# miroslavradojevic/pnr

Hardware: AMD Instinct MI355X
Metric: Mvox/s traced (Frangi+SMC step) on 1024^3 synthetic stack; % HBM roofline (higher is better)
Workload: dtype f32 (+f64 3x3 eigen-solver)

## Files before the change

### pnr_amd/csrc/api.cpp

```cpp
#include "ctx.h"
#include "replay.h"
#include "stream_sched.h"
#include "../host/reconstruct.h"
#include "recon.h"
#include "volume.h"
#include "radius.h"
#include "filter.h"
#include "distance.h"
#include <algorithm>
#include <cfloat>
#include <cmath>
#include <cstdlib>
#include <cstring>
#include <numeric>
#include <unordered_map>
#include <fstream>
#include <thread>
#include <sched.h>

namespace pnr {
static thread_local char g_err[512] = "";
void set_error(const char *fmt, ...)
{
    va_list ap;
// ... 964 lines not shown
    o.lag = std::max(-1, lag);
    pnr::SchedStats st;
    std::string err;
    const int rc = pnr::run_stream(eng, seeds, n, p->ni, o, sh, r, &st, err);
    if (rc) { set_error("%s", err.c_str()); return rc; }
    *n_nodes = (int64_t)r.nodes.size();
    *n_links = (int64_t)r.links.size() / 2;
    if (nodes) std::memcpy(nodes, r.nodes.data(), sizeof(pnr_node) * (size_t)std::min<int64_t>(cap_nodes, *n_nodes));
    if (links) std::memcpy(links, r.links.data(), 8 * (size_t)std::min<int64_t>(cap_links, *n_links));
    if (n_traces_used) *n_traces_used = r.trace_count;
    if (n_iterations) *n_iterations = st.iters;
    return PNR_OK;
}

namespace {
struct OptEntry { const char *key; int pnr::Options::*i32; int64_t pnr::Options::*i64; int64_t lo, hi; };
const OptEntry OPTS[] = {
    {"window", &pnr::Options::window, nullptr, 0, 1 << 20},      {"look0", &pnr::Options::look0, nullptr, 0, 1 << 24},
    {"look_pct", &pnr::Options::look_pct, nullptr, -1, 100000},   {"poll", &pnr::Options::poll, nullptr, 0, 1024},
    {"groups", &pnr::Options::groups, nullptr, 0, 4},            {"split_x10", &pnr::Options::split_x10, nullptr, 0, 10000},
    {"max_split", &pnr::Options::max_split, nullptr, 1, 4096},   {"stash_mb", nullptr, &pnr::Options::stash_mb, 1, 1 << 20},
    {"host_threads", &pnr::Options::host_threads, nullptr, 0, 1024}, {"local_ranks", &pnr::Options::local_ranks, nullptr, 1, 1024},
    {"trace_timing", &pnr::Options::trace_timing, nullptr, 0, 1}, {"seed_timing", &pnr::Options::seed_timing, nullptr, 0, 1},
    {"trace_log", &pnr::Options::trace_log, nullptr, 0, 1},
    {"replay_batches", &pnr::Options::replay_batches, nullptr, 0, 1}, {"batch_growth", &pnr::Options::batch_growth, nullptr, 100, 100000},
    {"batch_max", &pnr::Options::batch_max, nullptr, 1, 1 << 24}, {"no_stash", &pnr::Options::no_stash, nullptr, 0, 1},
    {"exchange_block", nullptr, &pnr::Options::exchange_block, 0, 1 << 28}, {"frangi_prune", &pnr::Options::frangi_prune, nullptr, 0, 1},
    {"cube_copy", &pnr::Options::cube_copy, nullptr, 0, 1},      {"gauss_march", &pnr::Options::gauss_march, nullptr, 0, 1},
    {"tentative", &pnr::Options::tentative, nullptr, 0, 1},      {"target", &pnr::Options::target, nullptr, -1, 1 << 20},
    {"sums_deep", &pnr::Options::sums_deep, nullptr, -1, 1},      {"sums_deep_max", &pnr::Options::sums_deep_max, nullptr, 0, 1 << 20},
    {"lag", &pnr::Options::lag, nullptr, -1, 1023},               {"profile_every", &pnr::Options::profile_every, nullptr, 1, 1024},
    {"overfill", &pnr::Options::overfill, nullptr, 0, 1},        {"concentrate", &pnr::Options::concentrate, nullptr, 0, 100},
    {"share_scales", &pnr::Options::share_scales, nullptr, 0, 1}, {"share_min", &pnr::Options::share_min, nullptr, 0, 1 << 20},
    {"hess_chunk", &pnr::Options::hess_chunk, nullptr, 0, 1 << 20},
    {"dist_split", &pnr::Options::dist_split, nullptr, 0, 1 << 22}, {"dist_pairs_per_launch", nullptr, &pnr::Options::dist_pairs_per_launch, 0, 1ll << 44},
};
}

int pnr_set_option(pnr_ctx *c, const char *key, int64_t value)
{
    PNR_REQUIRE(c && key, PNR_E_ARG, "null argument");
    if (std::strcmp(key, "recon_timing") == 0) {
        PNR_REQUIRE(value == 0 || value == 1, PNR_E_ARG, "option recon_timing = %lld outside [0, 1]", (long long)value);
        advantra::set_recon_timing(value != 0);
        return PNR_OK;
    }
    for (const OptEntry &e : OPTS)
        if (std::strcmp(e.key, key) == 0) {
            PNR_REQUIRE(value >= e.lo && value <= e.hi, PNR_E_ARG, "option %s = %lld outside [%lld, %lld]", key, (long long)value, (long long)e.lo, (long long)e.hi);
            if (e.i32) c->opt.*(e.i32) = (int)value; else c->opt.*(e.i64) = value;
            return PNR_OK;
        }
    set_error("unknown option '%s'", key);
    return PNR_E_ARG;
}

int pnr_get_option(pnr_ctx *c, const char *key, int64_t *value)
{
    PNR_REQUIRE(c && key && value, PNR_E_ARG, "null argument");
    if (std::strcmp(key, "recon_timing") == 0) { *value = advantra::recon_timing() ? 1 : 0; return PNR_OK; }
    if (std::strcmp(key, "host_threads_effective") == 0) { *value = pnr::host_threads(c->opt); return PNR_OK; }
    if (std::strcmp(key, "frangi_recomputes") == 0) { *value = c->frangi_recomputes; return PNR_OK; }
    for (const OptEntry &e : OPTS)
        if (std::strcmp(e.key, key) == 0) {
            *value = e.i32 ? (int64_t)(c->opt.*(e.i32)) : c->opt.*(e.i64);
            return PNR_OK;
        }
// ... 195 lines not shown
```

### pnr_amd/csrc/ctx.h

```cpp
#pragma once
#include "../../include/pnr_hip.h"
#include "../../include/pnr_hip_test.h"
#include "devbuf.h"
#include <hip/hip_runtime.h>
#include <algorithm>
#include <cstdarg>
#include <cstdio>
#include <map>
#include <string>
#include <unordered_map>
#include <vector>

namespace pnr {

void set_error(const char *fmt, ...);

#define PNR_HIP(call)                                                                        \
    do {                                                                                     \
        hipError_t e_ = (call);                                                              \
        if (e_ != hipSuccess) {                                                              \
            pnr::set_error("%s failed: %s (%s:%d)", #call, hipGetErrorString(e_), __FILE__, __LINE__); \
            return PNR_E_HIP;                                                                \
        }                                                                                    \
    } while (0)
// ... 33 lines not shown
void find_scale_pairs(Tables &t);
void glibc_rand_stream(uint32_t seed, int n, uint32_t *out);
int gaussian_taps(float sig, std::vector<float> &g);

struct Options {
    int window = 0;
    int look0 = 0, look_pct = -1;
    int target = -1;
    int sums_deep = -1;
    int sums_deep_max = 96;
    int lag = -1;
    int concentrate = 1;
    int overfill = 1;
    int poll = 0;
    int groups = 0;
    int split_x10 = 0;
    int max_split = 96;
    int64_t stash_mb = 65536;
    int host_threads = 0;
    int local_ranks = 1;
    int trace_timing = 0, seed_timing = 0;
    int profile_every = 1;
    int trace_log = 0;
    int replay_batches = 0;
    int batch_growth = 200, batch_max = 1024;
    int no_stash = 0;
    int frangi_prune = 1;
    int hess_chunk = 0;
    int tentative = 1;
    int gauss_march = 1;
    int cube_copy = 1;
    int share_scales = 1;
    int share_min = 0;
    int dist_split = 0;
    int64_t dist_pairs_per_launch = 0;
    int64_t exchange_block = 0;
};
int host_threads(const Options &o);

struct KernelTimer {
    double ms = 0;
    int64_t launches = 0;
};

}

struct pnr_ctx {
    pnr_params prm;
    pnr::Options opt;
    int device = 0;
    hipStream_t own_stream = nullptr, stream = nullptr;
    pnr::Tables tab;

    int64_t w = 0, h = 0, l = 0, N = 0;
    const uint8_t *d_img = nullptr;
    pnr::DevBuf<uint8_t> d_img_owned;

    pnr::DevBuf<float> d_tmpA, d_tmpB, d_J;
    pnr::DevBuf<uint8_t> d_Vx, d_Vy, d_Vz, d_J8;
    pnr::DevBuf<unsigned int> d_minmax;
    pnr::DevBuf<float> d_F[PNR_MAX_SIGMAS];
    pnr::DevBuf<uint8_t> d_scale;
    bool frangi_pruned = false, frangi_exact_once = false;
    float Jmax_run = 0.f;
    int64_t frangi_recomputes = 0;
    int64_t fr_zs0 = 0, fr_zs1 = 0;
// ... 160 lines not shown
```

### pnr_amd/csrc/smc_device.h

```cpp
#pragma once
#include "ctx.h"
#include <cfloat>
#include <cmath>

namespace {
typedef long long i64;
typedef float f32x2 __attribute__((ext_vector_type(2)));

struct Vol {
    const unsigned char *img;
    int w, h, l;
    i64 wh;
    float xmax, ymax, zmax;
};

struct Tab {
    const float *p, *u, *w0, *w0cws, *v, *w, *wcws;
    const float4 *tmpl;
    const int *M, *moff;
    const float *corrc, *sig;
    const unsigned int *rng;
    int sz, ndir, nsig, Mtot;
};

// ... 408 lines not shown
            const bool more = (iv * nu + iu + 1) < nv * nu;
            const float *nxt = more ? wk : wk - nw;
            r_wd = nxt[lane < nw ? lane : 0];
            for (int iw0 = 0; iw0 < nw; iw0 += G) {
                float xs[G], ys[G], zs[G];
#pragma unroll
                for (int j = 0; j < G; j++) {
                    const int iw = (iw0 + j < nw) ? iw0 + j : nw - 1;
                    const float ww = bcast(r_aw, iw);
                    const f32x2 xy = (f32x2){x1, y1} + (f32x2){ww, ww} * (f32x2){f.wx, f.wy};
                    xs[j] = xy.x;
                    ys[j] = xy.y;
                    zs[j] = z1 + ww * f.wz;
                }
                const Samples<G> sm = interp_group<G, CS>(V, B, xs, ys, zs);
#pragma unroll
                for (int j = 0; j < G; j++)
                    if (iw0 + j < nw) {
                        const float di = sm.v[j] - ag;
                        corra += di * bcast(r_cur, iw0 + j);
                        corrb = (float)((double)corrb + (double)di * (double)di);
                    }
            }
        }
    }
    }
    const float prod = corrb * corrc;
    return (prod > FLT_MIN) ? corra / sqrtf(prod) : 0.f;
}

template <int CS, bool IS2D = false, bool FAST = false, int PITCH = CS, bool INVOL = false>
__device__ __forceinline__ void sample_slice(const Vol &V, const Box &B, const Frame &f, int nv, int nu, int nw,
                                             const float *__restrict__ ax, int iv, float *__restrict__ stash_wave, int iu0 = 0,
                                             int iu1 = 1 << 30)
{
    constexpr int G = CHAIN_G;
    const int lane = threadIdx.x & 63;
    const float r_au = ax[nv + (lane < nu ? lane : 0)];
    const float r_aw = ax[nv + nu + (lane < nw ? lane : 0)];
    const float vv = ax[iv];
    const float x0 = f.px + vv * f.nvx, y0 = f.py + vv * f.nvy, z0 = f.pz + vv * f.nvz;
    if (iu1 > nu) iu1 = nu;
    typedef __attribute__((address_space(1))) float gfloat;
    gfloat *sp;
    {
        const unsigned long long a = (unsigned long long)(stash_wave + ((i64)iv * nu + iu0) * nw * 64);
        sp = (gfloat *)(((unsigned long long)(unsigned)__builtin_amdgcn_readfirstlane((int)(a >> 32)) << 32) | (unsigned)__builtin_amdgcn_readfirstlane((int)a));
    }
    const unsigned ulane = (unsigned)lane;
    for (int iu = iu0; iu < iu1; ++iu) {
        const float uu = bcast(r_au, iu);
        const float x1 = x0 + uu * f.ux, y1 = y0 + uu * f.uy, z1 = z0 + uu * f.uz;
        int iw0 = 0;
        for (; iw0 + G <= nw; iw0 += G) {
            float xs[G], ys[G], zs[G];
#pragma unroll
            for (int j = 0; j < G; j++) {
                const float ww = bcast(r_aw, iw0 + j);
                const f32x2 xy = (f32x2){x1, y1} + (f32x2){ww, ww} * (f32x2){f.wx, f.wy};
                xs[j] = xy.x;
                ys[j] = xy.y;
                zs[j] = z1 + ww * f.wz;
            }
            const Samples<G> sm = interp_group<G, CS, IS2D, FAST, PITCH, INVOL>(V, B, xs, ys, zs);
            gfloat *const pl = (sp + iw0 * 64) + ulane;
#pragma unroll
            for (int j = 0; j < G; j++) STASH_ST(&pl[j * 64], sm.v[j]);
        }
        if (iw0 < nw) {
            float xs[G], ys[G], zs[G];
#pragma unroll
            for (int j = 0; j < G; j++) {
                const int iw = (iw0 + j < nw) ? iw0 + j : nw - 1;
                const float ww = bcast(r_aw, iw);
                const f32x2 xy = (f32x2){x1, y1} + (f32x2){ww, ww} * (f32x2){f.wx, f.wy};
                xs[j] = xy.x;
                ys[j] = xy.y;
                zs[j] = z1 + ww * f.wz;
            }
            const Samples<G> sm = interp_group<G, CS, IS2D, FAST, PITCH, INVOL>(V, B, xs, ys, zs);
#pragma unroll
            for (int j = 0; j < G; j++)
                if (iw0 + j < nw) STASH_ST(&((sp + iw0 * 64) + ulane)[j * 64], sm.v[j]);
        }
        sp += nw * 64;
    }
}

template <int CS, bool IS2D = false, bool FAST = false, int PITCH = CS, bool INVOL = false>
__device__ __forceinline__ void sample_slice_packed(const Vol &V, const Box &B, const Frame &f, int nv, int nu, int nw,
                                                    const float *__restrict__ ax, int iv, int parts, int p, bool active,
                                                    float *__restrict__ stash_col, int stride, int r0 = 0, int r1 = 1 << 30)
{
    constexpr int G = CHAIN_G;
    const int lane = threadIdx.x & 63;
    const float r_au = ax[nv + (lane < nu ? lane : 0)];
    const float r_aw = ax[nv + nu + (lane < nw ? lane : 0)];
    const float vv = ax[iv];
    const float x0 = f.px + vv * f.nvx, y0 = f.py + vv * f.nvy, z0 = f.pz + vv * f.nvz;
    int rows = (nu + parts - 1) / parts;
    if (r1 < rows) rows = r1;
    for (int r = r0; r < rows; ++r) {
        const int iu = r * parts + p;
        const bool ok = active && iu < nu;
        const int iuc = iu < nu ? iu : nu - 1;
        const float uu = __shfl(r_au, iuc);
        const float x1 = x0 + uu * f.ux, y1 = y0 + uu * f.uy, z1 = z0 + uu * f.uz;
        float *sp = stash_col + ((i64)(iv * nu + iuc) * nw) * stride;
        int iw0 = 0;
        for (; iw0 + G <= nw; iw0 += G) {
            float xs[G], ys[G], zs[G];
#pragma unroll
            for (int j = 0; j < G; j++) {
                const float ww = bcast(r_aw, iw0 + j);
                const f32x2 xy = (f32x2){x1, y1} + (f32x2){ww, ww} * (f32x2){f.wx, f.wy};
                xs[j] = xy.x;
                ys[j] = xy.y;
                zs[j] = z1 + ww * f.wz;
            }
            const Samples<G> sm = interp_group<G, CS, IS2D, FAST, PITCH, INVOL>(V, B, xs, ys, zs);
            if (ok) {
#pragma unroll
                for (int j = 0; j < G; j++) STASH_ST(&sp[(iw0 + j) * stride], sm.v[j]);
            }
        }
        if (iw0 < nw) {
            float xs[G], ys[G], zs[G];
#pragma unroll
            for (int j = 0; j < G; j++) {
                const int iw = (iw0 + j < nw) ? iw0 + j : nw - 1;
                const float ww = bcast(r_aw, iw);
                const f32x2 xy = (f32x2){x1, y1} + (f32x2){ww, ww} * (f32x2){f.wx, f.wy};
                xs[j] = xy.x;
                ys[j] = xy.y;
                zs[j] = z1 + ww * f.wz;
            }
            const Samples<G> sm = interp_group<G, CS, IS2D, FAST, PITCH, INVOL>(V, B, xs, ys, zs);
#pragma unroll
            for (int j = 0; j < G; j++)
                if (ok && iw0 + j < nw) STASH_ST(&sp[(iw0 + j) * stride], sm.v[j]);
        }
    }
}

template <int STRIDE = 64, int CH = 32>
__device__ __forceinline__ float zncc_from_stash(const float *__restrict__ stash_lane, int M, const float *__restrict__ wd,
                                                 float corrc
#ifdef PNR_SMC_STAMPS
                                                 , unsigned long long *stamp_pass1 = nullptr
#endif
)
{
    const int nfull = M / CH, tail = M - nfull * CH;
    float cur[CH], nxt[CH];
    float ag = 0.f;
    if (nfull > 0) {
#pragma unroll
        for (int j = 0; j < CH; j++) cur[j] = STASH_LD(&stash_lane[j * STRIDE]);
    }
    for (int c = 0; c < nfull; c++) {
        const float *nx = stash_lane + (i64)(c + 1) * CH * STRIDE;
        if (c + 1 < nfull) {
#pragma unroll
            for (int j = 0; j < CH; j++) nxt[j] = STASH_LD(&nx[j * STRIDE]);
        }
#pragma unroll
        for (int j = 0; j < CH; j++) ag += cur[j];
#pragma unroll
        for (int j = 0; j < CH; j++) cur[j] = nxt[j];
    }
    {
        const float *tp = stash_lane + (i64)nfull * CH * STRIDE;
#pragma unroll
// ... 246 lines not shown
```

### pnr_amd/csrc/smc_phased.hip

```cpp
#include "ctx.h"
#include "replay.h"
#include "stream_sched.h"
#ifdef PNR_EXPERIMENT_HOOKS
#include "../../scripts/probes/experiments/ph_sample_hooks.h"
#else
#define PNR_HOOK_AFTER_FULL_ITEM(seg_lane, cnt)
#endif
#include "smc_device.h"
#include <algorithm>
#include <cstdlib>

namespace {

enum { FL_RES = 0, FL_STOP = 1, FL_T = 2, FL_IT = 3, FL_DONE = 4, FL_OX = 5, FL_OY = 6, FL_OZ = 7, FL_Y0 = 8, FL_Y1 = 9, FL_Z0 = 10, FL_Z1 = 11, FL_FAST = 12, FL_NCH = 13, FL_PAUSE = 14, FL_N = 16 };
constexpr int PH_THREADS = 1024;
constexpr int PH_CS = 54;
constexpr int PH_PITCH = 56;
constexpr int PH_PLANE = PH_CS * PH_PITCH;
static_assert((size_t)PH_CS * PH_PLANE <= 160 * 1024, "the cube must fit the LDS of a CU");

struct PhState {
    float *part;
    float *prior;
    int *idxres;
    float *corr;
    float *xcs;
    int *flags;
    float *stash;
    long long trace_floats;
    int stash_base;
    unsigned char *cubes;
    int *list;
    int *cnt;
    int *ctr;
    int *uidx;
    int *cmap;
    int cap;
    int np_pad;
    int W;
    int dedup;
};

__device__ __forceinline__ unsigned int pose_hash(float x, float y, float z, float vx, float vy, float vz)
// ... 309 lines not shown
                hs[k] = (unsigned int)c;
            }
            cbase += (int)__builtin_popcountll(m);
        }
        if (tid == 0) { uidx[cbase] = np; fl[FL_NCH] = cbase + 1; }
    }
    __syncthreads();
    for (int k = tid; k < np; k += B) cmap[k] = (int)hs[rep[k]];
#ifdef PNR_SMC_STAMPS
    if (tid == 0) {
        const unsigned long long pt6 = __builtin_amdgcn_s_memtime();
        atomicAdd(&g_pu_stamps[0], pt1 - pt0); atomicAdd(&g_pu_stamps[1], pt2 - pt1); atomicAdd(&g_pu_stamps[2], pt3 - pt2);
        atomicAdd(&g_pu_stamps[3], pt4 - pt3); atomicAdd(&g_pu_stamps[4], pt5 - pt4); atomicAdd(&g_pu_stamps[5], pt6 - pt5);
        atomicAdd(&g_pu_stamps[7], 1ull);
    }
#endif
}

constexpr int PH_CUBE_SPLIT = 16, PH_CUBE_THREADS = 256;
__global__ __launch_bounds__(PH_CUBE_THREADS) void ph_cube(Vol V, PhState P, int lp, int nslots)
{
    const int slot = blockIdx.x % nslots, part = blockIdx.x / nslots, tid = threadIdx.x;
    if (slot >= P.cnt[lp]) return;
    const int tr = P.list[lp * P.cap + slot];
    const int *fl = P.flags + (i64)tr * FL_N;
    if (fl[FL_PAUSE]) return;
    const CubeRows R = {fl[FL_OX], fl[FL_OY], fl[FL_OZ], fl[FL_Y0], fl[FL_Y1], fl[FL_Z0], fl[FL_Z1]};
    unsigned *dst = (unsigned *)(P.cubes + (i64)(P.stash_base + slot) * ((i64)PH_CS * PH_PLANE));
    stage_cube_rows(V, R, part * (PH_CUBE_THREADS >> 6) + (tid >> 6), PH_CUBE_SPLIT * (PH_CUBE_THREADS >> 6), tid & 63, dst);
}

#ifdef PNR_SMC_STAMPS
__device__ unsigned long long g_ph_stamps[8];
#endif

template <int CS, bool IS2D, bool GCUBE>
__global__ __launch_bounds__(PH_THREADS) __attribute__((amdgpu_waves_per_eu(5, 5))) void ph_sample(Vol V, Tab T, TabX X, PhState P, int np, int ni, int it_arg, int lp, int nslots, int share)
{
    extern __shared__ unsigned char cube[];
    const int slot = blockIdx.x % nslots, tid = threadIdx.x, B = blockDim.x, S = T.nsig;
    if (slot >= P.cnt[lp]) return;
    const int tr = P.list[lp * P.cap + slot];
    const int *fl = P.flags + (i64)tr * FL_N;
    if (fl[FL_PAUSE]) return;
    const int it = it_arg >= 0 ? it_arg : fl[FL_IT];
    const float *cur = P.part + (i64)tr * 2 * np * PSTRIDE + (it & 1) * np * PSTRIDE;
    const float *xc_pen = P.xcs + (i64)tr * 16 + ((it & 1) ^ 1) * 8;
    Box Bx;
    Bx.lds = (lds_cu8 *)cube;
    Bx.ox = fl[FL_OX]; Bx.oy = fl[FL_OY]; Bx.oz = fl[FL_OZ];
    Bx.org = (unsigned)(Bx.oz * PH_PLANE + Bx.oy * PH_PITCH + Bx.ox);
#ifdef PNR_SMC_STAMPS
    const unsigned long long st0 = __builtin_amdgcn_s_memtime();
    unsigned long long st_items = 0;
    if (Bx.ox + Bx.oy + Bx.oz + fl[FL_Y0] + fl[FL_Y1] + fl[FL_Z0] + fl[FL_Z1] == -12345) return;
    const unsigned long long st0b = __builtin_amdgcn_s_memtime();
#endif
    if constexpr (GCUBE) {
        static_assert(PH_PLANE % 16 == 0, "whole uint4 per plane");
        const int z0 = fl[FL_Z0], z1 = fl[FL_Z1];
        const uint4 *src = (const uint4 *)(P.cubes + (i64)(P.stash_base + slot) * ((i64)PH_CS * PH_PLANE) + (i64)z0 * PH_PLANE);
        uint4 *dst = (uint4 *)(cube + (size_t)z0 * PH_PLANE);
        const int n16 = (z1 - z0) * (PH_PLANE / 16);
        int i = tid;
        for (; i + 3 * B < n16; i += 4 * B) {
            const uint4 a0 = src[i], a1 = src[i + B], a2 = src[i + 2 * B], a3 = src[i + 3 * B];
            dst[i] = a0; dst[i + B] = a1; dst[i + 2 * B] = a2; dst[i + 3 * B] = a3;
        }
        for (; i < n16; i += B) dst[i] = src[i];
    } else {
        const CubeRows R = {Bx.ox, Bx.oy, Bx.oz, fl[FL_Y0], fl[FL_Y1], fl[FL_Z0], fl[FL_Z1]};
        stage_cube_rows(V, R, tid >> 6, B >> 6, tid & 63, (unsigned *)cube);
    }
    __syncthreads();
#ifdef PNR_SMC_STAMPS
    const unsigned long long st1 = __builtin_amdgcn_s_memtime();
#endif
    const int nch = __builtin_amdgcn_readfirstlane(fl[FL_NCH]);
    const int ngf = nch >> 6, rem = nch & 63, Rt = last_group_stride(rem);
    const int *uidx = P.uidx + (i64)tr * P.np_pad;
    const int fastword = __builtin_amdgcn_readfirstlane(fl[FL_FAST]);
    const int fastmask = fastword & 0xff;
    const int volmask = (fastword >> 8) & 0xff;
    constexpr int ROWS = 5;
    const int parts = rem > 0 ? 64 / rem : 1;
    const int skip = share ? X.guest_mask : 0;
    int nchsum = 0, npksum = 0;
    for (int s = 0; s < S; s++) {
        if (skip >> s & 1) continue;
        const int nv_s = __builtin_amdgcn_readfirstlane(X.grid[s].nv), nu_s = __builtin_amdgcn_readfirstlane(X.grid[s].nu);
        nchsum += nv_s * ((nu_s + ROWS - 1) / ROWS);
        npksum += nv_s * (((nu_s + parts - 1) / parts + ROWS - 1) / ROWS);
    }
    const int nfull = nchsum * ngf, nitems = nfull + (rem > 0 ? npksum : 0);
    float *const tbase = P.stash + (i64)(P.stash_base + slot) * P.trace_floats;
    const int lane = tid & 63;
    (void)ni;
    for (;;) {
        int item = 0;
        if (lane == 0) item = atomicAdd(&P.ctr[tr], 1);
        item = __builtin_amdgcn_readfirstlane(item);
        if (item >= nitems) break;
#ifdef PNR_SMC_STAMPS
        st_items++;
#endif
        const bool packed = item >= nfull;
        int sI = S - 1, r = packed ? item - nfull : item;
        while (sI > 0) {
            const int nv_s = __builtin_amdgcn_readfirstlane(X.grid[sI].nv), nu_s = __builtin_amdgcn_readfirstlane(X.grid[sI].nu);
            const int c = (skip >> sI & 1) ? 0 : packed ? nv_s * (((nu_s + parts - 1) / parts + ROWS - 1) / ROWS) : nv_s * ((nu_s + ROWS - 1) / ROWS) * ngf;
            if (r < c) break;
            r -= c;
            sI--;
        }
        const Grid gr = X.grid[sI];
        const int nv = __builtin_amdgcn_readfirstlane(gr.nv), nu = __builtin_amdgcn_readfirstlane(gr.nu);
        const int nw = __builtin_amdgcn_readfirstlane(gr.nw), goff = __builtin_amdgcn_readfirstlane(gr.off);
        const int Ms = nv * nu * nw;
        const float *ax = X.axes + __builtin_amdgcn_readfirstlane(X.axes_off[sI]);
        float *const sbase = tbase + (i64)goff * P.W;
        const int nch_rows = packed ? ((nu + parts - 1) / parts + ROWS - 1) / ROWS : (nu + ROWS - 1) / ROWS;
        const int per = packed ? nch_rows : nch_rows * ngf;
        const int iv = r / per, r2 = r - iv * per;
        if (!packed) {
            const int ch = r2 / ngf, g = r2 - ch * ngf;
            const int c = g * 64 + lane;
            const int k = uidx[c];
            const float *q = (k >= np) ? xc_pen : cur + k * PSTRIDE;
            const Frame f = make_frame(q[0], q[1], q[2], q[3], q[4], q[5]);
            bool item_fast = (fastmask >> sI & 1) != 0;
            if (!item_fast) {
                const int iu0 = ch * ROWS, iu1 = min(ch * ROWS + ROWS, nu) - 1;
                const float vv = ax[iv], uA = ax[nv + iu0], uB = ax[nv + iu1], wA = ax[nv + nu], wB = ax[nv + nu + nw - 1];
                const float bx = f.px + vv * f.nvx, by = f.py + vv * f.nvy, bz = f.pz + vv * f.nvz;
                bool ok = true;
                const float base[3] = {bx, by, bz}, ud[3] = {f.ux, f.uy, f.uz}, wd3[3] = {f.wx, f.wy, f.wz}, lim[3] = {V.xmax, V.ymax, V.zmax};
                const int org[3] = {Bx.ox, Bx.oy, Bx.oz};
#pragma unroll
                for (int a = 0; a < (IS2D ? 2 : 3); a++) {
                    const float c0 = (base[a] + uA * ud[a]) + wA * wd3[a], c1 = (base[a] + uA * ud[a]) + wB * wd3[a];
                    const float c2 = (base[a] + uB * ud[a]) + wA * wd3[a], c3 = (base[a] + uB * ud[a]) + wB * wd3[a];
                    const float lo = fminf(fminf(c0, c1), fminf(c2, c3)) - 1e-3f, hi = fmaxf(fmaxf(c0, c1), fmaxf(c2, c3)) + 1e-3f;
                    ok = ok && lo >= 0.f && hi <= lim[a] && floorf(lo) >= (float)org[a] && floorf(hi) + 1.f <= (float)(org[a] + CS - 1);
                }
                item_fast = __builtin_amdgcn_ballot_w64(!ok) == 0ull;
            }
#ifdef PNR_SMC_STAMPS
            if (lane == 0) atomicAdd(&g_pu_fine[item_fast ? 6 : 7], 1ull);
#endif
            if (item_fast)
                sample_slice<CS, IS2D, true, PH_PITCH>(V, Bx, f, nv, nu, nw, ax, iv, sbase + (i64)g * Ms * 64, ch * ROWS, ch * ROWS + ROWS);
            else if (volmask >> sI & 1)
                sample_slice<CS, IS2D, false, PH_PITCH, true>(V, Bx, f, nv, nu, nw, ax, iv, sbase + (i64)g * Ms * 64, ch * ROWS, ch * ROWS + ROWS);
            else
                sample_slice<CS, IS2D, false, PH_PITCH>(V, Bx, f, nv, nu, nw, ax, iv, sbase + (i64)g * Ms * 64, ch * ROWS, ch * ROWS + ROWS);
            PNR_HOOK_AFTER_FULL_ITEM(sbase + (i64)g * Ms * 64 + lane + ((i64)iv * nu + ch * ROWS) * nw * 64, (min(ch * ROWS + ROWS, nu) - ch * ROWS) * nw);
        } else {
            const bool act = lane < parts * rem;
            const int pp = act ? lane / rem : 0, j = act ? lane - pp * rem : 0;
            const int k = uidx[ngf * 64 + j];
            const float *q = (k >= np) ? xc_pen : cur + k * PSTRIDE;
            const Frame f = make_frame(q[0], q[1], q[2], q[3], q[4], q[5]);
            sample_slice_packed<CS, IS2D, false, PH_PITCH>(V, Bx, f, nv, nu, nw, ax, iv, parts, pp, act, sbase + (i64)ngf * Ms * 64 + j, Rt, r2 * ROWS, r2 * ROWS + ROWS);
        }
    }
#ifdef PNR_SMC_STAMPS
    if (tid == 0) {
        const unsigned long long st2 = __builtin_amdgcn_s_memtime();
        atomicAdd(&g_ph_stamps[0], st1 - st0);
        atomicAdd(&g_ph_stamps[4], st0b - st0);
        atomicAdd(&g_ph_stamps[1], st2 - st1);
        atomicAdd(&g_ph_stamps[2], 1ull);
        atomicAdd(&g_ph_stamps[3], st_items);
    }
#endif
}

constexpr int PH_CH = 32;
template <bool DEEP>
__global__ __launch_bounds__(64) void ph_sums(Tab T, TabX X, PhState P, int np, int np_pad, int ni, int it_arg, int lp, int ng_max, int share)
{
    const int S = T.nsig, lane = threadIdx.x;
    const int slot = blockIdx.x / (S * ng_max);
    if (slot >= P.cnt[lp]) return;
    const int tr = P.list[lp * P.cap + slot];
    const int *fl = P.flags + (i64)tr * FL_N;
    if (fl[FL_PAUSE]) return;
    const int r = blockIdx.x - slot * (S * ng_max);
    const int sI = r / ng_max, g = r - sI * ng_max;
    const int nch = fl[FL_NCH], ngf = nch >> 6, rem = nch & 63;
    if (g > ngf || (g == ngf && rem == 0)) return;
    (void)np; (void)ni; (void)it_arg;
    const Grid gr = X.grid[sI];
    const int M = gr.nv * gr.nu * gr.nw;
    const float *wd = X.wd + gr.off;
    const int host = (share && (X.guest_mask >> sI & 1)) ? X.share[sI] : -1;
    const Grid gh = X.grid[host >= 0 ? host : sI];
    const int Mh = gh.nv * gh.nu * gh.nw;
    const float *sbase = P.stash + (i64)(P.stash_base + slot) * P.trace_floats + (i64)gh.off * P.W;
    float cv;
    bool valid = true;
#ifdef PNR_SMC_STAMPS
    const unsigned long long sst0 = __builtin_amdgcn_s_memtime();
    unsigned long long sst1 = sst0;
#endif
    if (host >= 0) {
        const int *rows = X.grows + X.share[8 + sI];
// ... 352 lines not shown
    int stream_ni = 0;
    hipStream_t stg[MAXG] = {};
    hipEvent_t ev_start = nullptr;
    hipEvent_t ev_state[MAXG] = {};
    hipEvent_t ev_ctl[MAXG] = {};
};

static void phased_free(pnr_phased *h)
{
    h->state = {};
    h->d_s6.reset();
    h->out.reset();
    h->P = PhState{};
    h->O = TraceOut{};
    h->cap_traces = h->cap_dbg = 0;
    h->cap_stash = 0;
}

#ifdef PNR_SMC_STAMPS
extern "C" int pnr_debug_pu_fine(unsigned long long *out4, int reset)
{
    if (out4 && hipMemcpyFromSymbol(out4, HIP_SYMBOL(g_pu_fine), 64) != hipSuccess) return -1;
    if (reset) { unsigned long long z[8] = {}; if (hipMemcpyToSymbol(HIP_SYMBOL(g_pu_fine), z, 64) != hipSuccess) return -1; }
    return 0;
}

extern "C" int pnr_debug_pu_stamps(unsigned long long *out16, int reset)
{
    if (out16 && hipMemcpyFromSymbol(out16, HIP_SYMBOL(g_pu_stamps), 128) != hipSuccess) return -1;
    if (reset) { unsigned long long z[16] = {}; if (hipMemcpyToSymbol(HIP_SYMBOL(g_pu_stamps), z, 128) != hipSuccess) return -1; }
    return 0;
}

extern "C" int pnr_debug_ph_stamps(unsigned long long *out8, int reset)
{
    if (out8 && hipMemcpyFromSymbol(out8, HIP_SYMBOL(g_ph_stamps), 64) != hipSuccess) return -1;
    if (reset) { unsigned long long z[8] = {}; if (hipMemcpyToSymbol(HIP_SYMBOL(g_ph_stamps), z, 64) != hipSuccess) return -1; }
    return 0;
}
#endif

void pnr_phased_destroy(pnr_phased *h)
{
    if (!h) return;
    for (int r = 0; r < pnr_phased::RING; r++)
        if (h->ev[r]) (void)hipEventDestroy(h->ev[r]);
    for (int g = 1; g < pnr_phased::MAXG; g++)
        if (h->stg[g]) (void)hipStreamDestroy(h->stg[g]);
    if (h->ev_start) (void)hipEventDestroy(h->ev_start);
    for (hipEvent_t &e : h->ev_state) if (e) (void)hipEventDestroy(e);
    for (hipEvent_t &e : h->ev_ctl) if (e) (void)hipEventDestroy(e);
    delete h;
}

static bool sums_deep(const pnr_ctx *c, int active, int ngroups)
{
    if (c->opt.sums_deep >= 0) return c->opt.sums_deep != 0;
    return ngroups <= 1 || active <= c->opt.sums_deep_max;
}

static int share_scales(const pnr_ctx *c, int active)
{
    return (c->opt.share_scales && c->tab.guest_mask != 0 && active >= c->opt.share_min) ? 1 : 0;
}

static int ph_tbl(int np)
{
    int t = 64;
    while (t < 2 * np) t <<= 1;
    return t;
}

static size_t ph_predict_lds(int np, int dedup) { return dedup ? (size_t)(np * 8 + 2 * ph_tbl(np)) * 4 : (size_t)np * 8; }
// ... 119 lines not shown
        PNR_HIP(hipDeviceSynchronize());
        phased_free(h);
        const int64_t cap = NT;
        PNR_HIP(alloc_view(h->state.part, h->P.part, (size_t)cap * 2 * np * PSTRIDE));
        PNR_HIP(alloc_view(h->state.prior, h->P.prior, (size_t)cap * np));
        PNR_HIP(alloc_view(h->state.idxres, h->P.idxres, (size_t)cap * np));
        PNR_HIP(alloc_view(h->state.corr, h->P.corr, (size_t)cap * S * np_pad));
        PNR_HIP(alloc_view(h->state.xcs, h->P.xcs, (size_t)cap * 16));
        PNR_HIP(alloc_view(h->state.cnt, h->P.cnt, (size_t)cap * FL_N + 2 * pnr_phased::MAXG));
        h->P.flags = h->P.cnt + 2 * pnr_phased::MAXG;
        PNR_HIP(alloc_view(h->state.list, h->P.list, (size_t)cap * 2 * pnr_phased::MAXG));
        PNR_HIP(alloc_view(h->state.ctr, h->P.ctr, (size_t)cap));
        PNR_HIP(alloc_view(h->state.uidx, h->P.uidx, (size_t)cap * np_pad));
        PNR_HIP(alloc_view(h->state.cmap, h->P.cmap, (size_t)cap * np_pad));
        PNR_HIP(h->d_s6.alloc((size_t)cap * 6));
        PNR_HIP(alloc_view(h->out.T, h->O.T, (size_t)cap));
        PNR_HIP(alloc_view(h->out.stop, h->O.stop, (size_t)cap));
        PNR_HIP(alloc_view(h->out.xc, h->O.xc, (size_t)cap * ni * 8));
        const size_t dbg_cap = (size_t)cap * dbg_iters;
        if (dbg_iters && xfilt) PNR_HIP(alloc_view(h->out.xfilt, h->O.xfilt, dbg_cap * np * PSTRIDE));
        if (dbg_iters && idxres) PNR_HIP(alloc_view(h->out.idxres, h->O.idxres, dbg_cap * np));
        if (dbg_iters && neff) PNR_HIP(alloc_view(h->out.neff, h->O.neff, dbg_cap));
        h->cap_traces = cap; h->cap_dbg = (int64_t)dbg_cap;
        h->np = np; h->np_pad = np_pad; h->S = S; h->ni = ni; h->trace_floats = trace_floats;
        PNR_HIP(hipMemsetAsync(h->P.part, 0, (size_t)cap * 2 * np * PSTRIDE * 4, c->stream));
    }
    { const int rcs = ensure_stash(c, h, stash_want > 0 ? std::min<int64_t>(stash_want, NT) : NT, trace_floats); if (rcs) return rcs; }
    E.P = h->P;
    E.P.stash_base = 0;
    E.P.trace_floats = trace_floats;
    E.P.cap = (int)h->cap_traces;
    E.P.W = W;
    E.P.np_pad = np_pad;
    E.P.dedup = np <= 1024 ? 1 : 0;
    E.X.grid = (const Grid *)c->d_grid.get(); E.X.axes = c->d_axes.get(); E.X.axes_off = c->d_axes_off.get(); E.X.wd = c->d_wd.get();
    E.X.ext_v = c->tab.ext_v; E.X.ext_uw = c->tab.ext_uw;
    for (int s2 = 0; s2 < 8; s2++) { E.X.ext_vs[s2] = s2 < S ? c->tab.ext_vs[s2] : 0.f; E.X.ext_uws[s2] = s2 < S ? c->tab.ext_uws[s2] : 0.f; }
    E.X.stash = nullptr; E.X.slot_busy = nullptr; E.X.nslots = 0; E.X.slot_floats = 0; E.X.wave_floats = 0;
    E.X.share = c->d_share.get(); E.X.grows = c->d_grows.get(); E.X.guest_mask = c->tab.guest_mask;
    hipDeviceProp_t prop;
    PNR_HIP(hipGetDeviceProperties(&prop, c->device));
    E.ncu = prop.multiProcessorCount;
    E.np = np; E.ni = ni; E.S = S; E.np_pad = np_pad; E.ng = ngf + (rem > 0 ? 1 : 0); E.dbg_iters = dbg_iters;
    E.cube_bytes = (size_t)PH_CS * PH_PLANE;
    E.upd_lds = ((size_t)np * PSTRIDE + 4 * (size_t)np + (size_t)S * np_pad + 2 + 2 + 8) * 4;
    E.trace_floats = trace_floats;
    E.NT = NT;
    E.h = h;
    E.max_split = std::max(1, c->opt.max_split);
    PNR_REQUIRE(E.upd_lds <= 160 * 1024, PNR_E_ARG, "np=%d with %d scales needs %zu B of LDS in the update step (limit 160 KB)", np, S, E.upd_lds);
    PNR_HIP(hipFuncSetAttribute((const void *)ph_update, hipFuncAttributeMaxDynamicSharedMemorySize, (int)E.upd_lds));
    PNR_HIP(hipFuncSetAttribute((const void *)ph_sample<PH_CS, false, true>, hipFuncAttributeMaxDynamicSharedMemorySize, (int)E.cube_bytes));
    PNR_HIP(hipFuncSetAttribute((const void *)ph_sample<PH_CS, true, true>, hipFuncAttributeMaxDynamicSharedMemorySize, (int)E.cube_bytes));
    PNR_HIP(hipFuncSetAttribute((const void *)ph_sample<PH_CS, false, false>, hipFuncAttributeMaxDynamicSharedMemorySize, (int)E.cube_bytes));
    PNR_HIP(hipFuncSetAttribute((const void *)ph_sample<PH_CS, true, false>, hipFuncAttributeMaxDynamicSharedMemorySize, (int)E.cube_bytes));
    if (!c->opt.cube_copy) E.P.cubes = nullptr;
    return PNR_OK;
}

int pnr_trace_run_phased(pnr_ctx *c, const pnr_seed *seeds, int64_t n, int32_t *T_out, int32_t *stop_out, pnr_xest *xc, int dbg_iters,
                         float *xfilt, int32_t *idxres, float *neff, int use_density)
{
    if (n == 0) return PNR_OK;
    PhEnv E;
    const int64_t ntr_all = 2 * n;
    int rc = phased_env(c, ntr_all, dbg_iters, xfilt != nullptr, idxres != nullptr, neff != nullptr, E);
    if (rc) return rc;
// ... 292 lines not shown
```

### pnr_amd/lib.py

```python
import ctypes as C
import os
import subprocess
import numpy as np

HERE = os.path.dirname(os.path.abspath(__file__))
LIB_PATH = os.environ.get("PNR_LIB_DIAG") or os.path.join(HERE, "libpnr_hip.so")
PNR_MAX_SIGMAS = 8


class Window(C.Structure):
    _fields_ = [("lo", C.c_int32), ("hi", C.c_int32), ("sat_lo_ppm", C.c_int32), ("sat_hi_ppm", C.c_int32)]


def make_window(window):
    if window is None:
        return None
    if isinstance(window, dict):
        if set(window) != {"saturate"}:
            raise PnrError(f"window: (lo, hi) or {{'saturate': (lo_pct, hi_pct)}}, got {window!r}")
        a, b = window["saturate"]
        return Window(-1, -1, int(round(float(a) * 1e4)), int(round(float(b) * 1e4)))
    lo, hi = window
    return Window(int(lo), int(hi), 0, 0)

# ... 136 lines not shown
    L.pnr_sched_playback.argtypes = [C.POINTER(Params), i64, i64, i64, vp, i64, i32, i32, ALLGATHER_FN, vp, i64, TRACE_FN, vp, i32, i32, i32, i32, i32,
                                     vp, i64, C.POINTER(i64), vp, i64, C.POINTER(i64), C.POINTER(i64), C.POINTER(i64)]
    L.pnr_sched_playback2.argtypes = [C.POINTER(Params), i64, i64, i64, vp, i64, i32, i32, ALLGATHER_FN, vp, i64, TRACE_FN, vp, i32, i32, i32, i32, i32, i32, i32, i32,
                                      vp, i64, C.POINTER(i64), vp, i64, C.POINTER(i64), C.POINTER(i64), C.POINTER(i64)]
    L.pnr_get_trace_log.argtypes = [vp, vp, i64, C.POINTER(i64)]
    L.pnr_shm_exchange_open.argtypes = [C.c_char_p, i32, i32, i64, C.POINTER(vp)]
    L.pnr_shm_allgather.argtypes = [vp, vp, vp, i64]
    L.pnr_shm_exchange_close.argtypes = [vp]
    L.pnr_shm_exchange_close.restype = None
    L.pnr_rccl_unique_id.argtypes = [vp]
    L.pnr_rccl_exchange_open.argtypes = [vp, i32, i32, i32, i64, C.POINTER(vp)]
    L.pnr_rccl_allgather.argtypes = [vp, vp, vp, i64]
    L.pnr_rccl_allreduce_minmax.argtypes = [vp, C.POINTER(C.c_float), C.POINTER(C.c_float)]
    L.pnr_rccl_exchange_close.argtypes = [vp]
    L.pnr_rccl_exchange_close.restype = None
    L.pnr_set_option.argtypes = [vp, C.c_char_p, i64]
    L.pnr_get_option.argtypes = [vp, C.c_char_p, C.POINTER(i64)]
    for name in EXPORTS:
        if name not in ("pnr_last_error", "pnr_default_params", "pnr_destroy", "pnr_shm_exchange_close", "pnr_rccl_exchange_close"):
            getattr(L, name).restype = C.c_int
    _lib = L
    return L


PRODUCT_EXPORTS = ["pnr_last_error", "pnr_default_params", "pnr_create", "pnr_destroy", "pnr_set_stream", "pnr_synchronize",
                   "pnr_set_volume", "pnr_set_volume_device", "pnr_set_volume_u16", "pnr_set_volume_u16_device", "pnr_get_volume", "pnr_measure_radii", "pnr_filter_volume", "pnr_point_segment_distance", "pnr_tree_sample", "pnr_tree_distance", "pnr_frangi", "pnr_get_frangi", "pnr_extract_seeds", "pnr_extract_seeds_range",
                   "pnr_zncc_batch", "pnr_score_filter_sort_seeds", "pnr_trace_batch", "pnr_replay_traces", "pnr_replay_traces_ctx",
                   "pnr_frangi_slab", "pnr_quantise_j8", "pnr_soma", "pnr_get_soma", "pnr_trace_replay", "pnr_reconstruct", "pnr_reconstruct_ctx", "pnr_reconstruct_stage", "pnr_set_profiling",
                   "pnr_set_smc_driver", "pnr_get_kernel_ms", "pnr_reset_kernel_ms", "pnr_get_graph", "pnr_trace_replay_sharded",
                   "pnr_set_option", "pnr_get_option", "pnr_score_filter_seeds", "pnr_sort_seeds", "pnr_get_trace_log",
                   "pnr_shm_exchange_open", "pnr_shm_allgather", "pnr_shm_exchange_close",
                   "pnr_rccl_unique_id", "pnr_rccl_exchange_open", "pnr_rccl_allgather", "pnr_rccl_allreduce_minmax", "pnr_rccl_exchange_close"]
TEST_EXPORTS = ["pnr_gaussian", "pnr_hessian", "pnr_set_j8_v", "pnr_get_table", "pnr_expf_batch", "pnr_eigen_batch",
                "pnr_sched_playback", "pnr_sched_playback2", "pnr_reconstruct_stage_ctx", "pnr_radius_offsets", "pnr_live_bytes"]
EXPORTS = PRODUCT_EXPORTS + TEST_EXPORTS


def check(rc):
    if rc != 0:
        raise PnrError(f"libpnr_hip error {rc}: {load().pnr_last_error().decode()}")


def make_params(sigmas=(2, 4, 6), somaradius=0, tolerance=5, znccth=0.3, kappa=3, step=2, ni=200, np_=20, zdist=2,
                nodepervol=4, vol=1, rng_seed=42, **const):
    p = Params()
    load().pnr_default_params(C.byref(p))
    sig = sorted(float(s) for s in sigmas)
    if len(sig) > PNR_MAX_SIGMAS:
        raise PnrError("too many sigmas")
    for i, s in enumerate(sig):
        p.sig[i] = s
    p.nsig = len(sig)
    p.somaradius, p.tolerance, p.znccth, p.kappa = somaradius, tolerance, znccth, kappa
    p.step, p.ni, p.np, p.zdist, p.nodepervol, p.vol, p.rng_seed = step, ni, np_, zdist, nodepervol, vol, rng_seed
    for k, v in const.items():
        setattr(p, k, v)
    return p


DEFAULTS = {"smc_driver": None, "options": {}}


class Context:

    def __init__(self, params, device=0):
        self.L = load()
        self.p = params
# ... 477 lines not shown
    if count_only:
        return n.value
    pts = np.empty((n.value, 3), np.float32)
    owner = np.empty(n.value, np.int32)
    check(L.pnr_tree_sample(xyz.ctypes.data, parent.ctypes.data, len(xyz), float(zscale), float(step), pts.ctypes.data, owner.ctypes.data, n.value, C.byref(n)))
    return pts, owner


def read_swc(path):
    ids, xyz, par, index = [], [], [], {}
    with open(path) as f:
        for ln, line in enumerate(f, 1):
            t = line.split()
            if not t or t[0].startswith("#"):
                continue
            try:
                if len(t) < 7:
                    raise ValueError
                v = [float(x) for x in t[:7]]
                if not all(np.isfinite(v)) or v[0] != int(v[0]) or v[6] != int(v[6]):
                    raise ValueError
            except (ValueError, OverflowError):
                raise PnrError(f"{path}:{ln}: not an SWC line `n type x y z r parent`") from None
            if int(v[0]) in index:
                raise PnrError(f"{path}:{ln}: duplicate node id {int(v[0])}")
            index[int(v[0])] = len(ids)
            ids.append(int(v[0]))
            xyz.append(v[2:5])
            par.append(int(v[6]))
    parent = np.array([index.get(p, -1) if p >= 0 else -1 for p in par], np.int32).reshape(-1)
    return np.array(xyz, np.float64).reshape(-1, 3).astype(np.float32), parent, np.array(ids, np.int64).reshape(-1)


def live_bytes():
    dev, pin = C.c_int64(), C.c_int64()
    check(load().pnr_live_bytes(C.byref(dev), C.byref(pin)))
    return dev.value, pin.value


def radius_offsets(zdist, rmax, is2d=False):
    L = load()
    n = C.c_int64()
    starts = np.zeros(int(rmax) + 2 if 1 <= int(rmax) <= PNR_RADIUS_MAX else 2, np.int32)
    check(L.pnr_radius_offsets(float(zdist), int(rmax), int(bool(is2d)), starts.ctypes.data, None, None, None, 0, C.byref(n)))
    d = np.zeros((3, n.value), np.int32)
    check(L.pnr_radius_offsets(float(zdist), int(rmax), int(bool(is2d)), starts.ctypes.data, d[0].ctypes.data, d[1].ctypes.data, d[2].ctypes.data,
                               n.value, C.byref(n)))
    return starts, np.ascontiguousarray(d.T)


def reconstruct_stage(nodes, links, stage, trace_rsmpl=0.0, sig2radius=0.0, refine_iter=0, epsilon2=0.0, group_radius=0.0):
    L = load()
    nodes = np.ascontiguousarray(nodes, NODE_DT)
    links = np.ascontiguousarray(links, np.int32).reshape(-1, 2)
    L.pnr_reconstruct_stage.argtypes = [C.c_void_p, C.c_int64, C.c_void_p, C.c_int64, C.c_float, C.c_float, C.c_int, C.c_float, C.c_float, C.c_int,
                                        C.c_void_p, C.c_int64, C.POINTER(C.c_int64), C.c_void_p, C.c_int64, C.POINTER(C.c_int64)]
    nn, nl = C.c_int64(), C.c_int64()
    check(L.pnr_reconstruct_stage(nodes.ctypes.data, len(nodes), links.ctypes.data, len(links), trace_rsmpl, sig2radius, refine_iter, epsilon2,
                                  group_radius, stage, None, 0, C.byref(nn), None, 0, C.byref(nl)))
    out = np.zeros(nn.value, NODE_DT)
    lk = np.zeros((nl.value, 2), np.int32)
    check(L.pnr_reconstruct_stage(nodes.ctypes.data, len(nodes), links.ctypes.data, len(links), trace_rsmpl, sig2radius, refine_iter, epsilon2,
                                  group_radius, stage, out.ctypes.data, len(out), C.byref(nn), lk.ctypes.data, len(lk), C.byref(nl)))
    return out, lk


# ... 9 lines not shown
```

Measured before the change: 1353.

## Spread large packed remainder into full-width groups and specialise packed sampling paths

When the leftover particle group has more than 32 lanes, it is now treated as an extra full-width group using the regular per-lane slice sampler, with out-of-range lanes masked from storing. The packed sampler gains fast and in-volume template variants instead of always taking the generic path. Its stash addressing switches to a scalar base plus 32-bit offsets to cut address arithmetic. A dedup option, stash inspection API and extra timing counters are also added. The cost is more per-item bookkeeping and some wasted lane work in the extra group.

```diff
diff --git a/pnr_amd/csrc/api.cpp b/pnr_amd/csrc/api.cpp
--- a/pnr_amd/csrc/api.cpp
+++ b/pnr_amd/csrc/api.cpp
@@ -1020,7 +1020,7 @@
     {"lag", &pnr::Options::lag, nullptr, -1, 1023},               {"profile_every", &pnr::Options::profile_every, nullptr, 1, 1024},
     {"overfill", &pnr::Options::overfill, nullptr, 0, 1},        {"concentrate", &pnr::Options::concentrate, nullptr, 0, 100},
     {"share_scales", &pnr::Options::share_scales, nullptr, 0, 1}, {"share_min", &pnr::Options::share_min, nullptr, 0, 1 << 20},
-    {"hess_chunk", &pnr::Options::hess_chunk, nullptr, 0, 1 << 20},
+    {"hess_chunk", &pnr::Options::hess_chunk, nullptr, 0, 1 << 20}, {"dedup", &pnr::Options::dedup, nullptr, 0, 1},
     {"dist_split", &pnr::Options::dist_split, nullptr, 0, 1 << 22}, {"dist_pairs_per_launch", nullptr, &pnr::Options::dist_pairs_per_launch, 0, 1ll << 44},
 };
 }
diff --git a/pnr_amd/csrc/ctx.h b/pnr_amd/csrc/ctx.h
--- a/pnr_amd/csrc/ctx.h
+++ b/pnr_amd/csrc/ctx.h
@@ -89,6 +89,7 @@
     int cube_copy = 1;
     int share_scales = 1;
     int share_min = 0;
+    int dedup = 1;
     int dist_split = 0;
     int64_t dist_pairs_per_launch = 0;
     int64_t exchange_block = 0;
diff --git a/pnr_amd/csrc/smc_device.h b/pnr_amd/csrc/smc_device.h
--- a/pnr_amd/csrc/smc_device.h
+++ b/pnr_amd/csrc/smc_device.h
@@ -464,7 +464,7 @@
 template <int CS, bool IS2D = false, bool FAST = false, int PITCH = CS, bool INVOL = false>
 __device__ __forceinline__ void sample_slice(const Vol &V, const Box &B, const Frame &f, int nv, int nu, int nw,
                                              const float *__restrict__ ax, int iv, float *__restrict__ stash_wave, int iu0 = 0,
-                                             int iu1 = 1 << 30)
+                                             int iu1 = 1 << 30, bool store = true)
 {
     constexpr int G = CHAIN_G;
     const int lane = threadIdx.x & 63;
@@ -496,8 +496,10 @@
             }
             const Samples<G> sm = interp_group<G, CS, IS2D, FAST, PITCH, INVOL>(V, B, xs, ys, zs);
             gfloat *const pl = (sp + iw0 * 64) + ulane;
-#pragma unroll
-            for (int j = 0; j < G; j++) STASH_ST(&pl[j * 64], sm.v[j]);
+            if (store) {
+#pragma unroll
+                for (int j = 0; j < G; j++) STASH_ST(&pl[j * 64], sm.v[j]);
+            }
         }
         if (iw0 < nw) {
             float xs[G], ys[G], zs[G];
@@ -511,9 +513,11 @@
                 zs[j] = z1 + ww * f.wz;
             }
             const Samples<G> sm = interp_group<G, CS, IS2D, FAST, PITCH, INVOL>(V, B, xs, ys, zs);
-#pragma unroll
-            for (int j = 0; j < G; j++)
-                if (iw0 + j < nw) STASH_ST(&((sp + iw0 * 64) + ulane)[j * 64], sm.v[j]);
+            if (store) {
+#pragma unroll
+                for (int j = 0; j < G; j++)
+                    if (iw0 + j < nw) STASH_ST(&((sp + iw0 * 64) + ulane)[j * 64], sm.v[j]);
+            }
         }
         sp += nw * 64;
     }
@@ -522,7 +526,7 @@
 template <int CS, bool IS2D = false, bool FAST = false, int PITCH = CS, bool INVOL = false>
 __device__ __forceinline__ void sample_slice_packed(const Vol &V, const Box &B, const Frame &f, int nv, int nu, int nw,
                                                     const float *__restrict__ ax, int iv, int parts, int p, bool active,
-                                                    float *__restrict__ stash_col, int stride, int r0 = 0, int r1 = 1 << 30)
+                                                    float *__restrict__ stash_grp, int col, int stride, int r0 = 0, int r1 = 1 << 30)
 {
     constexpr int G = CHAIN_G;
     const int lane = threadIdx.x & 63;
@@ -530,6 +534,13 @@
     const float r_aw = ax[nv + nu + (lane < nw ? lane : 0)];
     const float vv = ax[iv];
     const float x0 = f.px + vv * f.nvx, y0 = f.py + vv * f.nvy, z0 = f.pz + vv * f.nvz;
+    typedef __attribute__((address_space(1))) float gfloat;
+    gfloat *sb;
+    {
+        const unsigned long long a = (unsigned long long)stash_grp;
+        sb = (gfloat *)(((unsigned long long)(unsigned)__builtin_amdgcn_readfirstlane((int)(a >> 32)) << 32) | (unsigned)__builtin_amdgcn_readfirstlane((int)a));
+    }
+    const unsigned ucol = (unsigned)col, ustride = (unsigned)stride;
     int rows = (nu + parts - 1) / parts;
     if (r1 < rows) rows = r1;
     for (int r = r0; r < rows; ++r) {
@@ -538,7 +549,7 @@
         const int iuc = iu < nu ? iu : nu - 1;
         const float uu = __shfl(r_au, iuc);
         const float x1 = x0 + uu * f.ux, y1 = y0 + uu * f.uy, z1 = z0 + uu * f.uz;
-        float *sp = stash_col + ((i64)(iv * nu + iuc) * nw) * stride;
+        const unsigned sp = (unsigned)((iv * nu + iuc) * nw) * ustride + ucol;
         int iw0 = 0;
         for (; iw0 + G <= nw; iw0 += G) {
             float xs[G], ys[G], zs[G];
@@ -553,7 +564,7 @@
             const Samples<G> sm = interp_group<G, CS, IS2D, FAST, PITCH, INVOL>(V, B, xs, ys, zs);
             if (ok) {
 #pragma unroll
-                for (int j = 0; j < G; j++) STASH_ST(&sp[(iw0 + j) * stride], sm.v[j]);
+                for (int j = 0; j < G; j++) STASH_ST(sb + (sp + (unsigned)(iw0 + j) * ustride), sm.v[j]);
             }
         }
         if (iw0 < nw) {
@@ -570,7 +581,7 @@
             const Samples<G> sm = interp_group<G, CS, IS2D, FAST, PITCH, INVOL>(V, B, xs, ys, zs);
 #pragma unroll
             for (int j = 0; j < G; j++)
-                if (ok && iw0 + j < nw) STASH_ST(&sp[(iw0 + j) * stride], sm.v[j]);
+                if (ok && iw0 + j < nw) STASH_ST(sb + (sp + (unsigned)(iw0 + j) * ustride), sm.v[j]);
         }
     }
 }
diff --git a/pnr_amd/csrc/smc_phased.hip b/pnr_amd/csrc/smc_phased.hip
--- a/pnr_amd/csrc/smc_phased.hip
+++ b/pnr_amd/csrc/smc_phased.hip
@@ -9,6 +9,7 @@
 #include "smc_device.h"
 #include <algorithm>
 #include <cstdlib>
+#include <cstring>
 
 namespace {
 
@@ -384,6 +385,7 @@
 
 #ifdef PNR_SMC_STAMPS
 __device__ unsigned long long g_ph_stamps[8];
+__device__ unsigned long long g_ph_last[16 + 64];
 #endif
 
 template <int CS, bool IS2D, bool GCUBE>
@@ -404,7 +406,7 @@
     Bx.org = (unsigned)(Bx.oz * PH_PLANE + Bx.oy * PH_PITCH + Bx.ox);
 #ifdef PNR_SMC_STAMPS
     const unsigned long long st0 = __builtin_amdgcn_s_memtime();
-    unsigned long long st_items = 0;
+    unsigned long long st_items = 0, lg_sum[9] = {};
     if (Bx.ox + Bx.oy + Bx.oz + fl[FL_Y0] + fl[FL_Y1] + fl[FL_Z0] + fl[FL_Z1] == -12345) return;
     const unsigned long long st0b = __builtin_amdgcn_s_memtime();
 #endif
@@ -436,6 +438,8 @@
     const int volmask = (fastword >> 8) & 0xff;
     constexpr int ROWS = 5;
     const int parts = rem > 0 ? 64 / rem : 1;
+    const bool spread = parts > 1;
+    const int ngs = ngf + (rem > 32 ? 1 : 0);
     const int skip = share ? X.guest_mask : 0;
     int nchsum = 0, npksum = 0;
     for (int s = 0; s < S; s++) {
@@ -444,7 +448,7 @@
         nchsum += nv_s * ((nu_s + ROWS - 1) / ROWS);
         npksum += nv_s * (((nu_s + parts - 1) / parts + ROWS - 1) / ROWS);
     }
-    const int nfull = nchsum * ngf, nitems = nfull + (rem > 0 ? npksum : 0);
+    const int nfull = nchsum * ngs, nitems = nfull + (spread ? npksum : 0);
     float *const tbase = P.stash + (i64)(P.stash_base + slot) * P.trace_floats;
     const int lane = tid & 63;
     (void)ni;
@@ -455,12 +459,15 @@
         if (item >= nitems) break;
 #ifdef PNR_SMC_STAMPS
         st_items++;
+        const unsigned long long lt0 = __builtin_amdgcn_s_memtime();
+        bool lg_item;
+        int lg_smp, lg_form;
 #endif
         const bool packed = item >= nfull;
         int sI = S - 1, r = packed ? item - nfull : item;
         while (sI > 0) {
             const int nv_s = __builtin_amdgcn_readfirstlane(X.grid[sI].nv), nu_s = __builtin_amdgcn_readfirstlane(X.grid[sI].nu);
-            const int c = (skip >> sI & 1) ? 0 : packed ? nv_s * (((nu_s + parts - 1) / parts + ROWS - 1) / ROWS) : nv_s * ((nu_s + ROWS - 1) / ROWS) * ngf;
+            const int c = (skip >> sI & 1) ? 0 : packed ? nv_s * (((nu_s + parts - 1) / parts + ROWS - 1) / ROWS) : nv_s * ((nu_s + ROWS - 1) / ROWS) * ngs;
             if (r < c) break;
             r -= c;
             sI--;
@@ -472,12 +479,13 @@
         const float *ax = X.axes + __builtin_amdgcn_readfirstlane(X.axes_off[sI]);
         float *const sbase = tbase + (i64)goff * P.W;
         const int nch_rows = packed ? ((nu + parts - 1) / parts + ROWS - 1) / ROWS : (nu + ROWS - 1) / ROWS;
-        const int per = packed ? nch_rows : nch_rows * ngf;
+        const int per = packed ? nch_rows : nch_rows * ngs;
         const int iv = r / per, r2 = r - iv * per;
         if (!packed) {
-            const int ch = r2 / ngf, g = r2 - ch * ngf;
+            const int ch = r2 / ngs, g = r2 - ch * ngs;
             const int c = g * 64 + lane;
-            const int k = uidx[c];
+            const bool live = c < nch;
+            const int k = uidx[live ? c : nch - 1];
             const float *q = (k >= np) ? xc_pen : cur + k * PSTRIDE;
             const Frame f = make_frame(q[0], q[1], q[2], q[3], q[4], q[5]);
             bool item_fast = (fastmask >> sI & 1) != 0;
@@ -498,14 +506,17 @@
                 item_fast = __builtin_amdgcn_ballot_w64(!ok) == 0ull;
             }
 #ifdef PNR_SMC_STAMPS
-            if (lane == 0) atomicAdd(&g_pu_fine[item_fast ? 6 : 7], 1ull);
+            lg_item = g == ngf;
+            if (lane == 0 && !lg_item) atomicAdd(&g_pu_fine[item_fast ? 6 : 7], 1ull);
+            lg_smp = (min(ch * ROWS + ROWS, nu) - ch * ROWS) * nw;
+            lg_form = item_fast ? 0 : (volmask >> sI & 1) ? 1 : 2;
 #endif
             if (item_fast)
-                sample_slice<CS, IS2D, true, PH_PITCH>(V, Bx, f, nv, nu, nw, ax, iv, sbase + (i64)g * Ms * 64, ch * ROWS, ch * ROWS + ROWS);
+                sample_slice<CS, IS2D, true, PH_PITCH>(V, Bx, f, nv, nu, nw, ax, iv, sbase + (i64)g * Ms * 64, ch * ROWS, ch * ROWS + ROWS, live);
             else if (volmask >> sI & 1)
-                sample_slice<CS, IS2D, false, PH_PITCH, true>(V, Bx, f, nv, nu, nw, ax, iv, sbase + (i64)g * Ms * 64, ch * ROWS, ch * ROWS + ROWS);
+                sample_slice<CS, IS2D, false, PH_PITCH, true>(V, Bx, f, nv, nu, nw, ax, iv, sbase + (i64)g * Ms * 64, ch * ROWS, ch * ROWS + ROWS, live);
             else
-                sample_slice<CS, IS2D, false, PH_PITCH>(V, Bx, f, nv, nu, nw, ax, iv, sbase + (i64)g * Ms * 64, ch * ROWS, ch * ROWS + ROWS);
+                sample_slice<CS, IS2D, false, PH_PITCH>(V, Bx, f, nv, nu, nw, ax, iv, sbase + (i64)g * Ms * 64, ch * ROWS, ch * ROWS + ROWS, live);
             PNR_HOOK_AFTER_FULL_ITEM(sbase + (i64)g * Ms * 64 + lane + ((i64)iv * nu + ch * ROWS) * nw * 64, (min(ch * ROWS + ROWS, nu) - ch * ROWS) * nw);
         } else {
             const bool act = lane < parts * rem;
@@ -513,8 +524,27 @@
             const int k = uidx[ngf * 64 + j];
             const float *q = (k >= np) ? xc_pen : cur + k * PSTRIDE;
             const Frame f = make_frame(q[0], q[1], q[2], q[3], q[4], q[5]);
-            sample_slice_packed<CS, IS2D, false, PH_PITCH>(V, Bx, f, nv, nu, nw, ax, iv, parts, pp, act, sbase + (i64)ngf * Ms * 64 + j, Rt, r2 * ROWS, r2 * ROWS + ROWS);
-        }
+            const bool item_fast = (fastmask >> sI & 1) != 0, item_invol = (volmask >> sI & 1) != 0;
+#ifdef PNR_SMC_STAMPS
+            lg_item = true;
+            lg_smp = (min(r2 * ROWS + ROWS, (nu + parts - 1) / parts) - r2 * ROWS) * nw;
+            lg_form = item_fast ? 0 : item_invol ? 1 : 2;
+#endif
+            float *const grp = sbase + (i64)ngf * Ms * 64;
+            if (item_fast)
+                sample_slice_packed<CS, IS2D, true, PH_PITCH>(V, Bx, f, nv, nu, nw, ax, iv, parts, pp, act, grp, j, Rt, r2 * ROWS, r2 * ROWS + ROWS);
+            else if (item_invol)
+                sample_slice_packed<CS, IS2D, false, PH_PITCH, true>(V, Bx, f, nv, nu, nw, ax, iv, parts, pp, act, grp, j, Rt, r2 * ROWS, r2 * ROWS + ROWS);
+            else
+                sample_slice_packed<CS, IS2D, false, PH_PITCH>(V, Bx, f, nv, nu, nw, ax, iv, parts, pp, act, grp, j, Rt, r2 * ROWS, r2 * ROWS + ROWS);
+        }
+#ifdef PNR_SMC_STAMPS
+        {
+            const unsigned long long dt = __builtin_amdgcn_s_memtime() - lt0;
+            lg_sum[lg_item ? 3 : 0] += 1; lg_sum[lg_item ? 4 : 1] += (unsigned long long)lg_smp; lg_sum[lg_item ? 5 : 2] += dt;
+            if (lg_item) lg_sum[6 + lg_form] += 1;
+        }
+#endif
     }
 #ifdef PNR_SMC_STAMPS
     if (tid == 0) {
@@ -524,7 +554,11 @@
         atomicAdd(&g_ph_stamps[1], st2 - st1);
         atomicAdd(&g_ph_stamps[2], 1ull);
         atomicAdd(&g_ph_stamps[3], st_items);
-    }
+        if ((int)blockIdx.x < nslots) atomicAdd(&g_ph_last[16 + rem], 1ull);
+    }
+    if (lane == 0)
+        for (int i = 0; i < 9; i++)
+            if (lg_sum[i]) atomicAdd(&g_ph_last[i], lg_sum[i]);
 #endif
 }
 
@@ -943,6 +977,13 @@
     return 0;
 }
 
+extern "C" int pnr_debug_ph_last(unsigned long long *out80, int reset)
+{
+    if (out80 && hipMemcpyFromSymbol(out80, HIP_SYMBOL(g_ph_last), 640) != hipSuccess) return -1;
+    if (reset) { unsigned long long z[80] = {}; if (hipMemcpyToSymbol(HIP_SYMBOL(g_ph_last), z, 640) != hipSuccess) return -1; }
+    return 0;
+}
+
 extern "C" int pnr_debug_ph_stamps(unsigned long long *out8, int reset)
 {
     if (out8 && hipMemcpyFromSymbol(out8, HIP_SYMBOL(g_ph_stamps), 64) != hipSuccess) return -1;
@@ -950,6 +991,27 @@
     return 0;
 }
 #endif
+
+extern "C" int pnr_phased_stash(pnr_ctx *c, int fill, float value, int64_t offset, int64_t n, float *out, int64_t *total, int64_t *trace_floats)
+{
+    PNR_REQUIRE(c, PNR_E_ARG, "null argument");
+    pnr_phased *h = c->phased;
+    PNR_REQUIRE(h && h->P.stash && h->cap_stash > 0, PNR_E_ARG, "no sample stash yet: run a trace call with the phased driver first");
+    const int64_t tot = h->cap_stash * (int64_t)h->trace_floats;
+    if (total) *total = tot;
+    if (trace_floats) *trace_floats = h->trace_floats;
+    PNR_HIP(hipDeviceSynchronize());
+    if (fill) {
+        unsigned bits;
+        std::memcpy(&bits, &value, 4);
+        PNR_HIP(hipMemsetD32(h->P.stash, (int)bits, (size_t)tot));
+    }
+    if (out) {
+        PNR_REQUIRE(offset >= 0 && n >= 0 && offset <= tot && n <= tot - offset, PNR_E_ARG, "stash range [%lld, +%lld) outside [0, %lld)", (long long)offset, (long long)n, (long long)tot);
+        PNR_HIP(hipMemcpy(out, h->P.stash + offset, (size_t)n * 4, hipMemcpyDeviceToHost));
+    }
+    return PNR_OK;
+}
 
 void pnr_phased_destroy(pnr_phased *h)
 {
@@ -1135,7 +1197,7 @@
     E.P.cap = (int)h->cap_traces;
     E.P.W = W;
     E.P.np_pad = np_pad;
-    E.P.dedup = np <= 1024 ? 1 : 0;
+    E.P.dedup = (np <= 1024 && c->opt.dedup) ? 1 : 0;
     E.X.grid = (const Grid *)c->d_grid.get(); E.X.axes = c->d_axes.get(); E.X.axes_off = c->d_axes_off.get(); E.X.wd = c->d_wd.get();
     E.X.ext_v = c->tab.ext_v; E.X.ext_uw = c->tab.ext_uw;
     for (int s2 = 0; s2 < 8; s2++) { E.X.ext_vs[s2] = s2 < S ? c->tab.ext_vs[s2] : 0.f; E.X.ext_uws[s2] = s2 < S ? c->tab.ext_uws[s2] : 0.f; }
diff --git a/pnr_amd/lib.py b/pnr_amd/lib.py
--- a/pnr_amd/lib.py
+++ b/pnr_amd/lib.py
@@ -192,7 +192,7 @@
                    "pnr_shm_exchange_open", "pnr_shm_allgather", "pnr_shm_exchange_close",
                    "pnr_rccl_unique_id", "pnr_rccl_exchange_open", "pnr_rccl_allgather", "pnr_rccl_allreduce_minmax", "pnr_rccl_exchange_close"]
 TEST_EXPORTS = ["pnr_gaussian", "pnr_hessian", "pnr_set_j8_v", "pnr_get_table", "pnr_expf_batch", "pnr_eigen_batch",
-                "pnr_sched_playback", "pnr_sched_playback2", "pnr_reconstruct_stage_ctx", "pnr_radius_offsets", "pnr_live_bytes"]
+                "pnr_sched_playback", "pnr_sched_playback2", "pnr_reconstruct_stage_ctx", "pnr_radius_offsets", "pnr_live_bytes", "pnr_phased_stash"]
 EXPORTS = PRODUCT_EXPORTS + TEST_EXPORTS
 
 
@@ -736,6 +736,15 @@
     return np.array(xyz, np.float64).reshape(-1, 3).astype(np.float32), parent, np.array(ids, np.int64).reshape(-1)
 
 
+def phased_stash(ctx, fill=None, offset=0, n=0):
+    L = load()
+    L.pnr_phased_stash.argtypes = [C.c_void_p, C.c_int32, C.c_float, C.c_int64, C.c_int64, C.c_void_p, C.POINTER(C.c_int64), C.POINTER(C.c_int64)]
+    out = np.zeros(n, np.float32)
+    total, per_trace = C.c_int64(), C.c_int64()
+    check(L.pnr_phased_stash(ctx.h, int(fill is not None), float(fill or 0.0), offset, n, out.ctypes.data if n else None, C.byref(total), C.byref(per_trace)))
+    return out, total.value, per_trace.value
+
+
 def live_bytes():
     dev, pin = C.c_int64(), C.c_int64()
     check(load().pnr_live_bytes(C.byref(dev), C.byref(pin)))
```

Result: no change. 1350 (median of 2 runs) (-0.3%).
